# levje/TrackToLearn

Measured on AMD Instinct MI355X. Metric: streamline-steps/s at n_actor=262144, higher is better.
Workload: dtype f32

## Files before the change

tracktolearn_amd/csrc/ttl_hip.hip:

```cpp
#include <hip/hip_runtime.h>

#include <algorithm>
#include <atomic>
#include <chrono>
#include <cmath>
#include <cstdarg>
#include <cstdio>
#include <cstdlib>
#include <cstring>
#include <new>
#include <type_traits>

#include "ttl_hip.h"

#include "ttl_internal.h"

#include <map>
#include <mutex>

namespace {
thread_local char g_err[512] = "";
}

int ttl_detail_fail(int code, const char *fmt, ...) {
// ... 1117 lines not shown
    const size_t nb = (n + BLOCK - 1) / BLOCK + 1;
    size_t end = 0;
    const auto rows = [&](auto *&region, size_t count, size_t per_row, size_t align = 256) {
        region = base ? reinterpret_cast<std::remove_reference_t<decltype(region)>>(
                            static_cast<char *>(base) + end) : nullptr;
        end += align_up(count * per_row, align);
    };
    rows(P.stop, n, 1);
    rows(P.rank, n, sizeof(int));
    rows(P.surv_pos, n, sizeof(int));
    rows(P.row_dest, n, sizeof(int));
    rows(P.block_counts, nb, sizeof(int));
    rows(P.proc_rank, n, sizeof(int));
    rows(P.proc_counts, nb, sizeof(int));
    rows(e.proc[0], n, sizeof(int));
    rows(e.proc[1], n, sizeof(int));
    rows(P.head, n, 4 * sizeof(float));
    rows(P.slot_head, n, 4 * sizeof(float));
    rows(P.last2, n, 8 * sizeof(float));
    rows(P.pos_dest, n, 2 * sizeof(int));
    rows(P.stop_list, n, 2 * sizeof(int));
    rows(P.slot_dest, n, sizeof(int));
    rows(P.counts, 64, sizeof(int));
    const size_t order_bytes = ttl_detail_order_workspace_bytes(n);
    static_assert(sizeof(ActRecord) <= 256 && alignof(ActRecord) <= 8, "see above");
    e.order_ws_bytes = order_bytes - 256;
    rows(e.order_ws, order_bytes, 1, 1);
    e.act_rec = e.order_ws ? reinterpret_cast<ActRecord *>(e.order_ws + e.order_ws_bytes) : nullptr;
    rows(e.ord_rec, n, sizeof(int2));
    rows(e.ord_count[0], 1, ttl_detail_order_instep_count_bytes());
    rows(e.ord_count[1], 1, ttl_detail_order_instep_count_bytes());
    return end;
}

static int knob(const char *name, int unset) {
    const char *v = getenv(name);
    return v ? atoi(v) : unset;
}
static void ttl_env_read_knobs(ttl_env &e) {
    EnvParams &P = e.P;
    const int rider_kinds[4] = {0, 3, 1, 2};
    e.proc_min_rows = knob("TTL_ORDER_MIN_ROWS", 8192);
    e.instep = std::max(knob("TTL_ORDER_INSTEP", 2), 0);
    e.instep_after = knob("TTL_ORDER_INSTEP_AFTER", 0) != 0;
    e.tail_riders = rider_kinds[knob("TTL_TAIL_RIDERS", 1) & 3];
    e.state_kernel = knob("TTL_STATE_KERNEL", 4);
    P.slot_rec = e.state_kernel != 2;
    P.xcd_remap = knob("TTL_XCD_REMAP", 1);
    P.xcd_rot = knob("TTL_XCD_ROTATE", 0) & 7;
    P.store_flavour = knob("TTL_STORE_FLAVOUR", 0);
    e.fuse_small = knob("TTL_FUSE_SMALL", 1);
    P.fuse_max_rows = std::clamp(knob("TTL_FUSE_MAX_ROWS", 64 * BLOCK), BLOCK, TTL_FUSE_MAX_BLOCKS * BLOCK);
    P.persist_rows = knob("TTL_GATHER_PERSIST_ROWS", 0);
    e.tail_fused = knob("TTL_TAIL_FUSED", 1);
    e.tail_fused_max = std::min(knob("TTL_TAIL_FUSED_MAX_ROWS", 262144), TTL_TAIL_MAX_BLOCKS * BLOCK);
    e.local_sort = knob("TTL_LOCAL_SORT", 1);
    e.poll_counts = knob("TTL_POLL_COUNTS", 1);
}

static int64_t state_width(const ttl_env_desc &d) { return 7LL * d.n_coef + 3LL * d.n_dirs; }

static int *idx_of(const ttl_env *env, int ahead = 0) {
    return (env->cur ^ ahead) ? env->d.idx_b : env->d.idx_a;
}

static void order_holds(ttl_env *env, int n) { env->use_proc = 1, env->n_slots = n; }
static void order_dropped(ttl_env *env) { env->use_proc = 0; }
static void order_rearmed(ttl_env *env, bool installed, int n) {
    env->proc_cur = env->ord_parity = 0;
    installed ? order_holds(env, n) : order_dropped(env);
}
static void order_compacted(ttl_env *env) { env->n_slots = -1; }
static void order_rebuilt(ttl_env *env) { env->ord_parity ^= 1, env->n_slots = -1; }
static void order_swapped(ttl_env *env) { env->proc_cur ^= env->use_proc ? 1 : 0; }
static int order_len(const ttl_env *env, int rows) { return env->n_slots < 0 ? rows : env->n_slots; }

extern "C" {

const char *ttl_last_error(void) { return g_err; }
uint32_t ttl_abi_version(void) { return TTL_ABI_VERSION; }
size_t ttl_env_desc_size(void) { return sizeof(ttl_env_desc); }

size_t ttl_env_workspace_bytes(int32_t n_max) {
    ttl_env sized;
    return n_max < 0 ? 0 : ttl_env_carve(sized, (size_t)n_max, nullptr);
}

int64_t ttl_sh_volume_records(const int32_t *dim, int32_t layout) {
    if (!dim || dim[0] < 1 || dim[1] < 1 || dim[2] < 1) return 0;
    if (layout == TTL_SH_BRICK4)
        return (int64_t)((dim[0] + 3) / 4) * ((dim[1] + 3) / 4) * ((dim[2] + 3) / 4) * 64;
    return (int64_t)dim[0] * dim[1] * dim[2];
}

struct VmmBlock {
    hipMemGenericAllocationHandle_t handle;
    size_t size;
};
static std::mutex g_vmm_mutex;
static std::map<void *, VmmBlock> g_vmm_blocks;

static hipError_t vmm_alloc(int device, size_t bytes, void **out) {
    hipMemAllocationProp prop{};
    prop.type = hipMemAllocationTypePinned;
    prop.location.type = hipMemLocationTypeDevice;
    prop.location.id = device;
// ... 991 lines not shown
```

tracktolearn_amd/csrc/ttl_internal.h:

```cpp
#ifndef TTL_INTERNAL_H
#define TTL_INTERNAL_H
#include <hip/hip_runtime.h>

#include <cstdint>

#include "ttl_hip.h"

int ttl_detail_fail(int code, const char *fmt, ...) __attribute__((format(printf, 2, 3)));
#define fail ttl_detail_fail

#define HIP_TRY(expr)                                                        \
    do {                                                                     \
        hipError_t e_ = (expr);                                              \
        if (e_ != hipSuccess)                                                \
            return fail(TTL_ERR_HIP, "%s: %s", #expr, hipGetErrorString(e_)); \
    } while (0)

constexpr int TTL_BLOCK = 256;

struct EnvParams {
    int mode;
    int sh_dim[3];
    int n_coef;
    int coef_pitch;
    const float *sh;
    float sh_shift;
    int sh_brick;
    unsigned sh_sx, sh_sy;
    int mask_dim[3];
    const double *mask_coef;
    const uint8_t *mask_cls;
    double mask_thr;
    int peaks_dim[3];
    const float *peaks;
    int compute_reward;
    float align_w;
    int n_dirs;
    int max_nb_steps;
    double step64;
    float step32;
    float radius;
    int curv_enabled;
    float curv_dot_max;
    float *hist;
    int *flags;
    int *lengths;
    uint8_t *dones;
    uint8_t *stop;
    float *head;
    int *pos_dest;
    float *last2;
    int *rank;
    int *surv_pos;
    int *row_dest;
    int *stop_list;
    int *block_counts;
    int *proc_rank;
    int *proc_counts;
    float *slot_head;
    int *slot_dest;
    int slot_rec;
    int store_flavour;
    int xcd_remap;
    int xcd_rot;
    int *counts;
    int fuse_max_rows;
    int persist_rows;
};

constexpr int TTL_FUSE_MAX_BLOCKS = 256;

constexpr int TTL_FR_LIVE = 8;
constexpr int TTL_FR_SNAP = 16;
constexpr int TTL_FR_NOISE = 32;

__device__ __forceinline__ void philox4x32_10(uint32_t &c0, uint32_t &c1, uint32_t &c2,
                                              uint32_t &c3, uint32_t k0, uint32_t k1) {
#pragma unroll
    for (int r = 0; r < 10; ++r) {
        const uint32_t hi0 = __umulhi(0xD2511F53u, c0), lo0 = 0xD2511F53u * c0;
        const uint32_t hi1 = __umulhi(0xCD9E8D57u, c2), lo1 = 0xCD9E8D57u * c2;
        c0 = hi1 ^ c1 ^ k0;
        c1 = lo1;
        c2 = hi0 ^ c3 ^ k1;
        c3 = lo0;
        k0 += 0x9E3779B9u;
        k1 += 0xBB67AE85u;
    }
}

struct FreerunView {
    const int *live, *idx_a, *idx_b;
    int cap;
};
void ttl_detail_freerun_view(const ttl_env *env, FreerunView *out);

__device__ __forceinline__ unsigned vox_x(const EnvParams &P, int x) {
    return P.sh_brick ? (unsigned)(x >> 2) * P.sh_sx + (unsigned)(x & 3) * 16u
                      : (unsigned)x * P.sh_sx;
}
__device__ __forceinline__ unsigned vox_y(const EnvParams &P, int y) {
    return P.sh_brick ? (unsigned)(y >> 2) * P.sh_sy + (unsigned)(y & 3) * 4u
                      : (unsigned)y * P.sh_sy;
}
__device__ __forceinline__ unsigned vox_z(const EnvParams &P, int z) {
    return P.sh_brick ? (unsigned)(z >> 2) * 64u + (unsigned)(z & 3) : (unsigned)z;
}

__device__ __forceinline__ int step_row_dest(int order, int row, bool stop, int pos, int total) {
    int dest = row;
    if (order == TTL_ORDER_PARTITION) dest = stop ? total + (row - pos) : pos;
    return dest;
}

__device__ __forceinline__ int step_map_row(const EnvParams &P, int row, int g, bool stop,
                                            int pos, int total, int order, int n_pts,
                                            int *idx_next) {
    const int dest = step_row_dest(order, row, stop, pos, total);
    if (!stop) idx_next[pos] = g;
    if (stop && order == TTL_ORDER_PARTITION) P.lengths[g] = n_pts;
// ... 519 lines not shown
```

tracktolearn_amd/csrc/ttl_state.hip:

```cpp
#include <type_traits>

#include "ttl_internal.h"


namespace {
constexpr int BLOCK = TTL_BLOCK;

template <int LPS>
struct LaneGroups {
    static constexpr int PER_WAVE = 64 / LPS;
    static constexpr int PER_BLOCK = (BLOCK / 64) * PER_WAVE;
    static dim3 grid(int n_rows) { return dim3((n_rows + PER_BLOCK - 1) / PER_BLOCK); }

    int grp, sub;
    __device__ LaneGroups() {
        const int lane = threadIdx.x & 63;
        grp = lane / LPS;
        sub = lane - grp * LPS;
    }
    __device__ bool idle() const { return grp >= PER_WAVE; }
    __device__ int slot(int blk) const {
        return blk * PER_BLOCK + (threadIdx.x >> 6) * PER_WAVE + grp;
    }
};

__device__ __forceinline__ const float *history_of(const EnvParams &P, int g) {
    return P.hist + (size_t)g * (size_t)(P.max_nb_steps + 1) * 3;
}

struct seg3 {
    float x, y, z;
};
__device__ __forceinline__ seg3 dir_segment(const float *__restrict__ h, int n_seg, int j) {
    seg3 v{0.0f, 0.0f, 0.0f};
    if (j < n_seg) {
        const float *a = h + (n_seg - 1 - j) * 3;
        const float ax = a[0], ay = a[1], az = a[2];
        const float bx = a[3], by = a[4], bz = a[5];
        v = seg3{bx - ax, by - ay, bz - az};
    }
    return v;
}
__device__ __forceinline__ void put_segment(float *__restrict__ od, int j, seg3 v) {
    od[3 * j + 0] = v.x;
    od[3 * j + 1] = v.y;
    od[3 * j + 2] = v.z;
}

template <int LPS>
__global__ __launch_bounds__(BLOCK) void k_state(
    EnvParams P, const int *__restrict__ idx, const int *__restrict__ row_dest,
    const int *__restrict__ proc, int n_rows, int L, float *__restrict__ out,
    long long pitch) {
#pragma clang fp contract(fast)
    const LaneGroups<LPS> lanes;
    const int slot = lanes.slot(blockIdx.x), sub = lanes.sub;
    if (lanes.idle() || slot >= n_rows) return;
    const int row = proc ? proc[slot] : slot;
    if (row < 0) return;
    const int g = idx ? idx[row] : row;
    const int r = row_dest ? row_dest[row] : row;
    const float *h = history_of(P, g);
    const float px = h[(L - 1) * 3 + 0];
    const float py = h[(L - 1) * 3 + 1];
    const float pz = h[(L - 1) * 3 + 2];
    float *orow = out + (size_t)r * (size_t)pitch;
    const int C = P.n_coef;
    const int C4 = P.coef_pitch >> 2;
    const int X = P.sh_dim[0], Y = P.sh_dim[1], Z = P.sh_dim[2];
    const float4 *vol = reinterpret_cast<const float4 *>(P.sh);

    for (int c4 = sub; c4 < C4; c4 += LPS) {
#pragma unroll
        for (int k = 0; k < 7; ++k) {
            const float ox = (k == 1) ? P.radius : (k == 4) ? -P.radius : 0.0f;
            const float oy = (k == 2) ? P.radius : (k == 5) ? -P.radius : 0.0f;
// ... 36 lines not shown
    a.comp = a.comp + v3.comp * w3;                                          \
    a.comp = a.comp + v4.comp * w4;                                          \
    a.comp = a.comp + v5.comp * w5;                                          \
    a.comp = a.comp + v6.comp * w6;                                          \
    a.comp = a.comp + v7.comp * w7;
            TTL_ACC(x) TTL_ACC(y) TTL_ACC(z) TTL_ACC(w)
#undef TTL_ACC
            const int c = c4 * 4;
            float *o = orow + k * C + c;
            if (c + 0 < C) o[0] = a.x;
            if (c + 1 < C) o[1] = a.y;
            if (c + 2 < C) o[2] = a.z;
            if (c + 3 < C) o[3] = a.w;
        }
    }
    float *od = orow + 7 * C;
    const int n_seg = L - 1;
    for (int j = sub; j < P.n_dirs; j += LPS) put_segment(od, j, dir_segment(h, n_seg, j));
}

struct f4 {
    float x, y, z, w;
};
__device__ __forceinline__ f4 ld4(const char *base, unsigned byte_off) {
    const float4 v = *reinterpret_cast<const float4 *>(base + byte_off);
    return f4{v.x, v.y, v.z, v.w};
}
__device__ __forceinline__ f4 scale4(f4 a, float w) {
    return f4{a.x * w, a.y * w, a.z * w, a.w * w};
}
__device__ __forceinline__ f4 fma4(f4 a, float w, f4 c) {
    return f4{__builtin_fmaf(a.x, w, c.x), __builtin_fmaf(a.y, w, c.y),
              __builtin_fmaf(a.z, w, c.z), __builtin_fmaf(a.w, w, c.w)};
}
__device__ __forceinline__ f4 sel4(bool c, f4 a, f4 b) {
    return f4{c ? a.x : b.x, c ? a.y : b.y, c ? a.z : b.z, c ? a.w : b.w};
}
template <bool OUTER>
__device__ __forceinline__ f4 blend(f4 v00, f4 v01, f4 v10, f4 v11, float a0, float a1,
                                    float b0, float b1) {
    f4 r = OUTER ? fma4(v00, a0 * b0, scale4(v01, a0 * b1))
                 : fma4(v01, a0 * b1, scale4(v00, a0 * b0));
    r = fma4(v10, a1 * b0, r);
    return fma4(v11, a1 * b1, r);
}
template <bool MINUS>
__device__ __forceinline__ f4 lerp(f4 lo, f4 hi, float d) {
    return MINUS ? fma4(hi, d, scale4(lo, 1.0f - d)) : fma4(lo, 1.0f - d, scale4(hi, d));
}
struct AxisPoints {
    f4 centre, plus, minus;
};
__device__ __forceinline__ AxisPoints stencil_axis(
    const char *vol, const f4 (&lo)[4], const f4 (&hi)[4], const unsigned (&q)[4], unsigned below,
    unsigned above, float a0, float a1, float b0, float b1, bool dn, bool up, float d,
    float d_plus, float d_minus) {
    const f4 zero{0.f, 0.f, 0.f, 0.f};
    f4 s0 = zero, s3 = zero;
    if (dn)
        s0 = blend<true>(ld4(vol, below + q[0]), ld4(vol, below + q[1]), ld4(vol, below + q[2]),
                         ld4(vol, below + q[3]), a0, a1, b0, b1);
    if (up)
        s3 = blend<true>(ld4(vol, above + q[0]), ld4(vol, above + q[1]), ld4(vol, above + q[2]),
                         ld4(vol, above + q[3]), a0, a1, b0, b1);
    const f4 s1 = blend<false>(lo[0], lo[1], lo[2], lo[3], a0, a1, b0, b1);
    const f4 s2 = blend<false>(hi[0], hi[1], hi[2], hi[3], a0, a1, b0, b1);
    return AxisPoints{lerp<false>(s1, s2, d),
                      lerp<false>(sel4(up, s2, s1), sel4(up, s3, s2), d_plus),
                      lerp<true>(sel4(dn, s0, s1), sel4(dn, s1, s2), d_minus)};
}
__device__ __forceinline__ int clipi(int v, int n) { return min(max(v, 0), n - 1); }
typedef float v4f __attribute__((ext_vector_type(4)));
typedef v4f v4f_dword_aligned __attribute__((aligned(4)));
__device__ __forceinline__ float from_prev_lane(float v) {
    return __int_as_float(
        __builtin_amdgcn_update_dpp(0, __float_as_int(v), 0x111, 0xf, 0xf, false));
}
__device__ __forceinline__ void store16(float *o, v4f v, int flavour) {
    if (flavour == 0) {
        *reinterpret_cast<v4f_dword_aligned *>(o) = v;
    } else if (flavour == 1) {
        asm volatile("global_store_dwordx4 %0, %1, off sc1" : : "v"(o), "v"(v) : "memory");
    } else if (flavour == 2) {
        asm volatile("global_store_dwordx4 %0, %1, off nt" : : "v"(o), "v"(v) : "memory");
    } else {
        asm volatile("global_store_dwordx4 %0, %1, off sc0 sc1" : : "v"(o), "v"(v) : "memory");
    }
}

template <bool MERGE_TAIL>
__device__ __forceinline__ void put4(int flavour, float *o, f4 a, int c, int C) {
    if (MERGE_TAIL && (flavour & 8)) {
        const int rem = C & 3;
        const bool last = c + 3 >= C;
        v4f v{a.x, a.y, a.z, a.w};
        int back = 0;
        if (rem == 1) {
            const float py = from_prev_lane(a.y), pz = from_prev_lane(a.z), pw = from_prev_lane(a.w);
            if (last) v = v4f{py, pz, pw, a.x};
            back = last ? 3 : 0;
        } else if (rem == 2) {
            const float pz = from_prev_lane(a.z), pw = from_prev_lane(a.w);
            if (last) v = v4f{pz, pw, a.x, a.y};
            back = last ? 2 : 0;
        } else if (rem == 3) {
            const float pw = from_prev_lane(a.w);
            if (last) v = v4f{pw, a.x, a.y, a.z};
            back = last ? 1 : 0;
        }
        store16(o - back, v, flavour & 7);
        return;
    }
    if (MERGE_TAIL) {
        const f4 p{from_prev_lane(a.x), from_prev_lane(a.y), from_prev_lane(a.z),
                   from_prev_lane(a.w)};
        const int back = (c + 3 < C) ? 0 : 4 - (C - c);
        v4f v{a.x, a.y, a.z, a.w};
        if (back == 1) v = v4f{p.w, a.x, a.y, a.z};
        if (back == 2) v = v4f{p.z, p.w, a.x, a.y};
        if (back == 3) v = v4f{p.y, p.z, p.w, a.x};
        store16(o - back, v, flavour);
        return;
    }
    if (c + 3 < C) {
        store16(o, v4f{a.x, a.y, a.z, a.w}, flavour);
    } else {
        if (c + 0 < C) o[0] = a.x;
        if (c + 1 < C) o[1] = a.y;
        if (c + 2 < C) o[2] = a.z;
    }
}

template <int LPS, bool LOOP, bool MERGE_TAIL>
__device__ __forceinline__ void state_row_dd(const EnvParams &P, float px, float py,
                                             float pz, const float *__restrict__ h, int L,
                                             int sub, float *__restrict__ orow) {
    const seg3 first_dir = sub < P.n_dirs ? dir_segment(h, L - 1, sub) : seg3{0.0f, 0.0f, 0.0f};
    const int C = P.n_coef;
    const int C4 = P.coef_pitch >> 2;
    const int X = P.sh_dim[0], Y = P.sh_dim[1], Z = P.sh_dim[2];
    const char *vol = reinterpret_cast<const char *>(P.sh);
    const float rad = P.radius;

    float cxp = px + rad, cxm = px + (-rad);
    float cyp = py + rad, cym = py + (-rad);
    float czp = pz + rad, czm = pz + (-rad);
    if (P.sh_shift != 0.0f) {
        px += P.sh_shift; py += P.sh_shift; pz += P.sh_shift;
        cxp += P.sh_shift; cxm += P.sh_shift;
        cyp += P.sh_shift; cym += P.sh_shift;
        czp += P.sh_shift; czm += P.sh_shift;
    }
    const float fx = floorf(px), fy = floorf(py), fz = floorf(pz);
    const float dx = px - fx, dy = py - fy, dz = pz - fz;
    const float ex = 1.0f - dx, ey = 1.0f - dy, ez = 1.0f - dz;
    const float fxp = floorf(cxp), fxm = floorf(cxm);
    const float fyp = floorf(cyp), fym = floorf(cym);
    const float fzp = floorf(czp), fzm = floorf(czm);
    const float dxp = cxp - fxp, dxm = cxm - fxm;
    const float dyp = cyp - fyp, dym = cym - fym;
    const float dzp = czp - fzp, dzm = czm - fzm;
    const bool xup = fxp > fx, xdn = fxm < fx;
    const bool yup = fyp > fy, ydn = fym < fy;
    const bool zup = fzp > fz, zdn = fzm < fz;
    const int ix = (int)fminf(fmaxf(fx, -4.0f), (float)X + 4.0f);
    const int iy = (int)fminf(fmaxf(fy, -4.0f), (float)Y + 4.0f);
    const int iz = (int)fminf(fmaxf(fz, -4.0f), (float)Z + 4.0f);
    const unsigned rec = (unsigned)C4 * 16u;
    const unsigned x0 = vox_x(P, clipi(ix - 1, X)) * rec, x1 = vox_x(P, clipi(ix, X)) * rec,
                   x2 = vox_x(P, clipi(ix + 1, X)) * rec, x3 = vox_x(P, clipi(ix + 2, X)) * rec;
    const unsigned y0 = vox_y(P, clipi(iy - 1, Y)) * rec, y1 = vox_y(P, clipi(iy, Y)) * rec,
                   y2 = vox_y(P, clipi(iy + 1, Y)) * rec, y3 = vox_y(P, clipi(iy + 2, Y)) * rec;
    const unsigned z0 = vox_z(P, clipi(iz - 1, Z)) * rec, z1 = vox_z(P, clipi(iz, Z)) * rec,
                   z2 = vox_z(P, clipi(iz + 1, Z)) * rec, z3 = vox_z(P, clipi(iz + 2, Z)) * rec;
    for (int c4 = sub; c4 < C4; c4 += LPS) {
        const unsigned cb = (unsigned)c4 * 16u;
        const int c = c4 * 4;
        const unsigned qx[4] = {y1 + z1 + cb, y1 + z2 + cb, y2 + z1 + cb, y2 + z2 + cb};
        const unsigned qy[4] = {x1 + z1 + cb, x1 + z2 + cb, x2 + z1 + cb, x2 + z2 + cb};
        const unsigned qz[4] = {x1 + y1 + cb, x1 + y2 + cb, x2 + y1 + cb, x2 + y2 + cb};
        const f4 v000 = ld4(vol, x1 + qx[0]), v001 = ld4(vol, x1 + qx[1]);
        const f4 v010 = ld4(vol, x1 + qx[2]), v011 = ld4(vol, x1 + qx[3]);
        const f4 v100 = ld4(vol, x2 + qx[0]), v101 = ld4(vol, x2 + qx[1]);
        const f4 v110 = ld4(vol, x2 + qx[2]), v111 = ld4(vol, x2 + qx[3]);
        const AxisPoints ax = stencil_axis(vol, {v000, v001, v010, v011}, {v100, v101, v110, v111},
                                           qx, x0, x3, ey, dy, ez, dz, xdn, xup, dx, dxp, dxm);
        put4<MERGE_TAIL>(P.store_flavour, orow + 0 * C + c, ax.centre, c, C);
        put4<MERGE_TAIL>(P.store_flavour, orow + 1 * C + c, ax.plus, c, C);
        put4<MERGE_TAIL>(P.store_flavour, orow + 4 * C + c, ax.minus, c, C);
        const AxisPoints ay = stencil_axis(vol, {v000, v001, v100, v101}, {v010, v011, v110, v111},
                                           qy, y0, y3, ex, dx, ez, dz, ydn, yup, dy, dyp, dym);
        put4<MERGE_TAIL>(P.store_flavour, orow + 2 * C + c, ay.plus, c, C);
        put4<MERGE_TAIL>(P.store_flavour, orow + 5 * C + c, ay.minus, c, C);
        const AxisPoints az = stencil_axis(vol, {v000, v010, v100, v110}, {v001, v011, v101, v111},
                                           qz, z0, z3, ex, dx, ey, dy, zdn, zup, dz, dzp, dzm);
        put4<MERGE_TAIL>(P.store_flavour, orow + 3 * C + c, az.plus, c, C);
        put4<MERGE_TAIL>(P.store_flavour, orow + 6 * C + c, az.minus, c, C);
        if (!LOOP) break;
    }
    float *od = orow + 7 * C;
    if (sub < P.n_dirs) put_segment(od, sub, first_dir);
    for (int j = sub + LPS; j < P.n_dirs; j += LPS)
        put_segment(od, j, dir_segment(h, L - 1, j));
}

__device__ __forceinline__ void tail_rider(const EnvParams &P, const TailRiders &R, int wg) {
    if (wg < R.n_scatter) {
        extern __shared__ unsigned s_rider[];
        order_scatter_block(s_rider, wg, R.n_scatter, R.rec, R.n_slots, R.count, R.count_other,
                            R.bins, R.order_out);
        return;
    }
    wg -= R.n_scatter;
    const int i = wg * BLOCK + threadIdx.x;
    if (wg >= R.n_row_blocks || i >= R.n_active) return;
    step_map_row(P, i, R.idx[i], P.stop[i] != 0, R.row_base[wg] + P.rank[i], P.counts[0],
                 R.order, R.n_pts, R.idx_next);
}

__device__ __forceinline__ int xcd_block(const EnvParams &P, int blk, int nwg) {
    const int q = nwg >> 3, rr = nwg & 7, xcd = blk & 7;
    if (P.xcd_rot == 0)
        return (xcd < rr ? xcd * (q + 1) : rr * (q + 1) + (xcd - rr) * q) + (blk >> 3);
    const int mine = (xcd + P.xcd_rot) & 7;
    int start = 0;
    for (int r = 0; r < mine; ++r) start += q + ((((r - P.xcd_rot) & 7) < rr) ? 1 : 0);
    return start + (blk >> 3);
}

struct SlotRow {
    int g, r;
    float px, py, pz;
    const float *h;
};
__device__ __forceinline__ bool resolve_slot(const EnvParams &P, const int *__restrict__ idx,
                                             const int *__restrict__ row_dest,
                                             const int *__restrict__ proc, int slot, int L,
                                             SlotRow &s) {
    if (proc && idx && P.slot_rec) {
        const float4 hp = *reinterpret_cast<const float4 *>(P.slot_head + 4 * (size_t)slot);
        s = SlotRow{__float_as_int(hp.w), P.slot_dest[slot], hp.x, hp.y, hp.z, nullptr};
        if (s.r < 0) return false;
        s.h = history_of(P, s.g);
        return true;
    }
    const int row = proc ? proc[slot] : slot;
    if (row < 0) return false;
    s.g = idx ? idx[row] : row;
    s.r = row_dest ? row_dest[row] : row;
    s.h = history_of(P, s.g);
    if (idx) {
        const float4 hp = *reinterpret_cast<const float4 *>(P.head + 4 * (size_t)row);
        s.px = hp.x;
        s.py = hp.y;
        s.pz = hp.z;
    } else {
        s.px = s.h[(L - 1) * 3 + 0];
        s.py = s.h[(L - 1) * 3 + 1];
        s.pz = s.h[(L - 1) * 3 + 2];
    }
    return true;
}

template <int LPS, int MINW, bool LOOP, bool MERGE_TAIL>
__global__ __launch_bounds__(BLOCK, MINW) void k_state_dd(
    EnvParams P, const int *__restrict__ idx, const int *__restrict__ row_dest,
    const int *__restrict__ proc, int n_rows, int L, float *__restrict__ out,
    long long pitch, int n_vblocks, TailRiders riders) {
    if ((int)blockIdx.x >= n_vblocks) {
        tail_rider(P, riders, (int)blockIdx.x - n_vblocks);
        return;
    }
    const LaneGroups<LPS> lanes;
    if (lanes.idle()) return;
    for (int vb = blockIdx.x; vb < n_vblocks; vb += gridDim.x) {
        const int slot = lanes.slot(proc && P.xcd_remap ? xcd_block(P, vb, n_vblocks) : vb);
        SlotRow s;
        if (slot >= n_rows || !resolve_slot(P, idx, row_dest, proc, slot, L, s)) continue;
        state_row_dd<LPS, LOOP, MERGE_TAIL>(P, s.px, s.py, s.pz, s.h, L, lanes.sub,
                                            out + (size_t)s.r * (size_t)pitch);
    }
}

template <int LPS, bool MERGE_TAIL, bool FR>
__device__ __forceinline__ void prefix_state_body(
    const EnvParams &P, const int *__restrict__ idx, int *__restrict__ idx_next, int n_active,
    int n_blocks, int order, int n_pts, float *__restrict__ out, long long pitch,
    int *__restrict__ host_word, int seq, int cur) {
    __shared__ int s_before[TTL_FUSE_MAX_BLOCKS + 1];
    const int lane = threadIdx.x & 63;
    if (threadIdx.x < 64) {
        int c[4];
#pragma unroll
        for (int k = 0; k < 4; ++k)
            c[k] = 4 * lane + k < n_blocks ? P.block_counts[4 * lane + k] : 0;
        const int local = (c[0] + c[1]) + (c[2] + c[3]);
        int v = local;
#pragma unroll
        for (int off = 1; off < 64; off <<= 1) {
            const int t = __shfl_up(v, off);
            if (lane >= off) v += t;
        }
        int run = v - local;
#pragma unroll
        for (int k = 0; k < 4; ++k) {
            s_before[4 * lane + k] = run;
            run += c[k];
        }
        if (lane == 63) s_before[TTL_FUSE_MAX_BLOCKS] = v;
    }
    __syncthreads();
    const int total = s_before[TTL_FUSE_MAX_BLOCKS];
    if (blockIdx.x == 0 && threadIdx.x == 0) {
        if (FR) {
            int *live = P.counts + TTL_FR_LIVE;
            live[0] = total;
            live[1] = n_active > 0 ? n_pts : n_pts - 1;
            live[2] = n_active > 0 ? cur ^ 1 : cur;
            live[3] = seq;
        }
        step_publish_counts(P, total, n_active, host_word, seq);
    }
    const LaneGroups<LPS> lanes;
    const int row = lanes.slot(blockIdx.x), sub = lanes.sub;
    if (lanes.idle() || row >= n_active) return;
    const float4 hp = *reinterpret_cast<const float4 *>(P.head + 4 * (size_t)row);
    const int g = __float_as_int(hp.w);
    const bool stop = P.stop[row] != 0;
    const int pos = s_before[row >> 8] + P.rank[row];
    const int dest = step_row_dest(order, row, stop, pos, total);
    if (sub == 0) step_map_row(P, row, g, stop, pos, total, order, n_pts, idx_next);
    state_row_dd<LPS, false, MERGE_TAIL>(P, hp.x, hp.y, hp.z, history_of(P, g), n_pts, sub,
                                         out + (size_t)dest * (size_t)pitch);
}

template <int LPS, bool MERGE_TAIL>
__global__ __launch_bounds__(BLOCK, 4) void k_prefix_state(
    EnvParams P, const int *__restrict__ idx, int *__restrict__ idx_next, int n_active,
    int n_blocks, int order, int n_pts, float *__restrict__ out, long long pitch,
    int *__restrict__ host_word, int seq) {
    prefix_state_body<LPS, MERGE_TAIL, false>(P, idx, idx_next, n_active, n_blocks, order,
                                              n_pts, out, pitch, host_word, seq, 0);
}

template <int LPS, bool MERGE_TAIL>
__global__ __launch_bounds__(BLOCK, 4) void k_prefix_state_fr(
    EnvParams P, int *__restrict__ idx_a, int *__restrict__ idx_b, int n_blocks,
    float *__restrict__ out, long long pitch, int *__restrict__ host_word) {
    const int *snap = P.counts + TTL_FR_SNAP;
    const int n_active = snap[0], L = snap[1], cur = snap[2], seq = snap[3] + 1;
    if (snap[4]) {
        if (blockIdx.x == 0 && threadIdx.x == 0) {
            P.counts[TTL_FR_LIVE + 3] = seq;
            if (host_word)
                __hip_atomic_store(host_word + 2, seq, __ATOMIC_RELEASE, __HIP_MEMORY_SCOPE_SYSTEM);
        }
        return;
    }
    prefix_state_body<LPS, MERGE_TAIL, true>(P, cur ? idx_b : idx_a, cur ? idx_a : idx_b,
                                             n_active, n_blocks, TTL_ORDER_PARTITION, L + 1,
                                             out, pitch, host_word, seq, cur);
}

template <int MAX_LPS, class F>
void for_lanes_per_streamline(const EnvParams &P, F &&f) {
    const int C4 = P.coef_pitch >> 2;
    const bool tail_straddles = C4 == 9 && (P.n_coef & 3);
    if (C4 <= 4) f(std::integral_constant<int, 4>{});
    else if (C4 <= 8) f(std::integral_constant<int, 8>{});
    else if (C4 <= 12 && !tail_straddles) f(std::integral_constant<int, 12>{});
    else if (MAX_LPS == 16 || C4 <= 16) f(std::integral_constant<int, 16>{});
    else f(std::integral_constant<int, MAX_LPS>{});
}

bool dedupe_applies(const EnvParams &P) {
    const size_t vol_bytes = ttl_detail_sh_records(P) * P.coef_pitch * sizeof(float);
    return P.radius > 0.0f && P.radius < 1.0f && vol_bytes < (1ull << 32);
}

}

bool ttl_detail_can_fuse_tail(const EnvParams &P, int n_active) {
    const int C4 = P.coef_pitch >> 2;
    return n_active <= P.fuse_max_rows && dedupe_applies(P) && C4 <= 16 && P.n_coef >= 4;
}

int ttl_detail_launch_fused_tail(const EnvParams &P, const int *idx, int *idx_next,
                                 int n_active, int order, int n_pts, float *out,
                                 int64_t pitch, int *host_word, int seq, hipStream_t s) {
    const int n_blocks = (n_active + BLOCK - 1) / BLOCK;
    for_lanes_per_streamline<16>(P, [&](auto lps) {
        constexpr int LPS = decltype(lps)::value;
        hipLaunchKernelGGL((k_prefix_state<LPS, true>), LaneGroups<LPS>::grid(n_active), dim3(BLOCK), 0,
                           s, P, idx, idx_next, n_active, n_blocks, order, n_pts, out,
                           (long long)pitch, host_word, seq);
    });
    HIP_TRY(hipGetLastError());
    return TTL_OK;
}

int ttl_detail_launch_fused_tail_fr(const EnvParams &P, int *idx_a, int *idx_b, int n_cap,
                                    float *out, int64_t pitch, int *host_word,
                                    hipStream_t s) {
    const int n_blocks = (n_cap + BLOCK - 1) / BLOCK;
    for_lanes_per_streamline<16>(P, [&](auto lps) {
        constexpr int LPS = decltype(lps)::value;
        hipLaunchKernelGGL((k_prefix_state_fr<LPS, true>), LaneGroups<LPS>::grid(n_cap), dim3(BLOCK), 0,
                           s, P, idx_a, idx_b, n_blocks, out, (long long)pitch, host_word);
    });
    HIP_TRY(hipGetLastError());
    return TTL_OK;
}

bool ttl_detail_state_dedupes(const EnvParams &P, int state_kernel) {
    return state_kernel != 0 && dedupe_applies(P);
}

int ttl_detail_launch_state(const EnvParams &P, int state_kernel, const int *idx,
                            const int *row_dest, const int *proc, int n_rows, int L,
                            float *out, int64_t pitch, hipStream_t s,
                            const TailRiders *riders) {
    const bool dedupe = ttl_detail_state_dedupes(P, state_kernel);
    const TailRiders R = riders ? *riders : TailRiders{};
    const int n_riders = R.n_scatter + R.n_row_blocks;
    const size_t lds = R.n_scatter ? ttl_detail_order_scatter_lds(R.bins) : 0;
    if (n_riders && (!dedupe || P.persist_rows > 0 || lds > TTL_RIDER_MAX_LDS))
        return fail(TTL_ERR_INVALID, "state gather: this launch cannot carry riders");
    for_lanes_per_streamline<32>(P, [&](auto lps) {
        constexpr int LPS = decltype(lps)::value;
        const int n_vb = (int)LaneGroups<LPS>::grid(n_rows).x;
        const int resident = 1024;
        const bool persist = dedupe && n_rows <= P.persist_rows && n_vb > resident;
        const dim3 grid(persist ? resident : n_vb + n_riders);
        if (!dedupe)
            hipLaunchKernelGGL((k_state<LPS>), grid, dim3(BLOCK), 0, s, P, idx, row_dest, proc,
                               n_rows, L, out, (long long)pitch);
        else if constexpr (LPS < 32) {
            if (P.n_coef >= 4 && state_kernel != 3)
                hipLaunchKernelGGL((k_state_dd<LPS, 4, false, true>), grid, dim3(BLOCK), lds, s, P,
                                   idx, row_dest, proc, n_rows, L, out, (long long)pitch, n_vb, R);
            else
                hipLaunchKernelGGL((k_state_dd<LPS, 4, false, false>), grid, dim3(BLOCK), lds, s, P,
                                   idx, row_dest, proc, n_rows, L, out, (long long)pitch, n_vb, R);
        } else {
            hipLaunchKernelGGL((k_state_dd<LPS, 2, true, false>), grid, dim3(BLOCK), lds, s, P, idx,
                               row_dest, proc, n_rows, L, out, (long long)pitch, n_vb, R);
        }
    });
    HIP_TRY(hipGetLastError());
    return TTL_OK;
}
```

Baseline: 909.5 million.

## Restage state gather row to cut register pressure and pin waves per SIMD

Measured after the change: 912.5 million (median of 4 runs). About the same (+0.3%).

```diff
diff --git a/profiles/state_occupancy_resources.py b/profiles/state_occupancy_resources.py
--- /dev/null
+++ b/profiles/state_occupancy_resources.py
@@ -0,0 +1,124 @@
+#!/usr/bin/env python
+import argparse
+import importlib.util
+import os
+import re
+import subprocess
+import sys
+import tempfile
+
+ROOT = os.path.dirname(os.path.dirname(os.path.abspath(__file__)))
+TABLE = os.path.join(ROOT, 'profiles', 'state_occupancy_resource_usage.md')
+UNIT = 'tracktolearn_amd/csrc/ttl_state.hip'
+COLUMNS = ('SGPRs', 'SGPRs spilled', 'VGPRs', 'VGPRs spilled', 'scratch B/lane',
+           'waves/SIMD', 'LDS B/block')
+_REMARK = {'TotalSGPRs': 'SGPRs', 'SGPRs Spill': 'SGPRs spilled', 'VGPRs': 'VGPRs',
+           'VGPRs Spill': 'VGPRs spilled', 'ScratchSize': 'scratch B/lane',
+           'Occupancy': 'waves/SIMD', 'LDS Size': 'LDS B/block'}
+
+
+def _build_module():
+    spec = importlib.util.spec_from_file_location(
+        'ttl_csrc_build', os.path.join(ROOT, 'tracktolearn_amd', 'csrc', 'build.py'))
+    mod = importlib.util.module_from_spec(spec)
+    spec.loader.exec_module(mod)
+    return mod
+
+
+def kernel_name(mangled):
+    m = re.match(r'_ZN12_GLOBAL__N_1(\d+)', mangled)
+    if not m:
+        return mangled
+    start = m.end()
+    name = mangled[start:start + int(m.group(1))]
+    rest = mangled[start + int(m.group(1)):]
+    args = []
+    if rest.startswith('I'):
+        for kind, value in re.findall(r'L([ib])(n?\d+)E', rest[1:rest.index('EE') + 1]):
+            args.append(('false', 'true')[int(value)] if kind == 'b' else value.replace('n', '-'))
+    return f'{name}<{", ".join(args)}>' if args else name
+
+
+def report(tree=ROOT):
+    build = _build_module()
+    flags = [f for f in build.FLAGS if f not in ('-shared', '-fPIC')]
+    with tempfile.TemporaryDirectory() as tmp:
+        cmd = [build.find_hipcc()] + flags + [
+            '-Rpass-analysis=kernel-resource-usage', '--cuda-device-only',
+            '-I', os.path.join(tree, 'include'), '-I', os.path.join(tree, 'tracktolearn_amd', 'csrc'),
+            '-c', os.path.join(tree, UNIT), '-o', os.path.join(tmp, 'ttl_state.o')]
+        err = subprocess.run(cmd, check=True, stderr=subprocess.PIPE, text=True).stderr
+    kernels, cur = {}, None
+    for line in err.splitlines():
+        m = re.search(r'remark: +(.*?)(?: \[-Rpass-analysis=kernel-resource-usage\])?$', line)
+        if not m:
+            continue
+        text = m.group(1)
+        m = re.match(r'Function Name: (\S+)', text)
+        if m:
+            cur = kernels.setdefault(kernel_name(m.group(1)), {})
+            continue
+        m = re.match(r'([A-Za-z ]+?)(?: \[[^\]]*\])?: (\d+)$', text)
+        if m and cur is not None and m.group(1) in _REMARK:
+            cur[_REMARK[m.group(1)]] = int(m.group(2))
+    return kernels
+
+
+def table(kernels):
+    lines = ['| kernel | ' + ' | '.join(COLUMNS) + ' |', '|---' * (len(COLUMNS) + 1) + '|']
+    for name, row in kernels.items():
+        lines.append(f'| `{name}` | ' + ' | '.join(str(row[c]) for c in COLUMNS) + ' |')
+    return '\n'.join(lines)
+
+
+def read_table(heading, path=TABLE):
+    kernels, inside = {}, False
+    with open(path) as f:
+        for line in f:
+            if line.startswith('## '):
+                inside = line[3:].strip() == heading
+            m = re.match(r'\| `([^`]+)` \|(.*)\|\s*$', line)
+            if inside and m:
+                kernels[m.group(1)] = dict(zip(COLUMNS, (int(v) for v in m.group(2).split('|'))))
+    return kernels
+
+
+def parent_tree(rev, tmp):
+    for path in ('include', 'tracktolearn_amd/csrc'):
+        tar = subprocess.run(['git', '-C', ROOT, 'archive', rev, path], check=True,
+                             stdout=subprocess.PIPE).stdout
+        subprocess.run(['tar', '-x', '-C', tmp], input=tar, check=True)
+    return tmp
+
+
+HEADER = '''# State gather: registers, scratch and waves per SIMD (DESIGN 3.1, 4.1)
+
+The compiler's report (`-Rpass-analysis=kernel-resource-usage`) of every kernel of
+`tracktolearn_amd/csrc/ttl_state.hip`, compiled alone and device side only with the flags of
+`tracktolearn_amd/csrc/build.py`; written by `profiles/state_occupancy_resources.py`, runs without
+a GPU.  "Parent" is the commit before the row of `state_row_dd` was restated in four stages (the
+centre cell reduced to its six blended slices at once, then one axis at a time with its own
+geometry); "This tree" is the source next to this file.  The second template argument of
+`k_state_dd` is the waves per SIMD the instantiation is held to (`amdgpu_waves_per_eu`, both
+bounds; `TTL_GATHER_WAVES` picks 4, 5 or 6 for the one-column gather): where the body needs fewer
+registers than that bound allows, the kernel descriptor is padded to it, so "waves/SIMD" is what
+the hardware will keep resident.  `tests/test_state_kernel_resources.py` holds this tree to the
+table below: no instantiation may gain scratch, and the 5-wave gather has none.
+'''
+
+
+def main():
+    ap = argparse.ArgumentParser(description=__doc__.split('\n')[0])
+    ap.add_argument('--parent', default='HEAD~1', help='revision of the parent tree')
+    args = ap.parse_args()
+    with tempfile.TemporaryDirectory() as tmp:
+        parent = report(parent_tree(args.parent, tmp))
+    rev = subprocess.run(['git', '-C', ROOT, 'rev-parse', '--short', args.parent], check=True,
+                         stdout=subprocess.PIPE, text=True).stdout.strip()
+    with open(TABLE, 'w') as f:
+        f.write(f'{HEADER}\n## Parent\n\n(`{rev}`)\n\n{table(parent)}\n\n## This tree\n\n{table(report())}\n')
+    print(TABLE)
+
+
+if __name__ == '__main__':
+    sys.exit(main())
diff --git a/tracktolearn_amd/csrc/ttl_hip.hip b/tracktolearn_amd/csrc/ttl_hip.hip
--- a/tracktolearn_amd/csrc/ttl_hip.hip
+++ b/tracktolearn_amd/csrc/ttl_hip.hip
@@ -1193,6 +1193,7 @@
     e.fuse_small = knob("TTL_FUSE_SMALL", 1);
     P.fuse_max_rows = std::clamp(knob("TTL_FUSE_MAX_ROWS", 64 * BLOCK), BLOCK, TTL_FUSE_MAX_BLOCKS * BLOCK);
     P.persist_rows = knob("TTL_GATHER_PERSIST_ROWS", 0);
+    P.gather_waves = std::clamp(knob("TTL_GATHER_WAVES", 4), 4, 6);
     e.tail_fused = knob("TTL_TAIL_FUSED", 1);
     e.tail_fused_max = std::min(knob("TTL_TAIL_FUSED_MAX_ROWS", 262144), TTL_TAIL_MAX_BLOCKS * BLOCK);
     e.local_sort = knob("TTL_LOCAL_SORT", 1);
diff --git a/tracktolearn_amd/csrc/ttl_internal.h b/tracktolearn_amd/csrc/ttl_internal.h
--- a/tracktolearn_amd/csrc/ttl_internal.h
+++ b/tracktolearn_amd/csrc/ttl_internal.h
@@ -66,6 +66,7 @@
     int *counts;
     int fuse_max_rows;
     int persist_rows;
+    int gather_waves;
 };
 
 constexpr int TTL_FUSE_MAX_BLOCKS = 256;
diff --git a/tracktolearn_amd/csrc/ttl_state.hip b/tracktolearn_amd/csrc/ttl_state.hip
--- a/tracktolearn_amd/csrc/ttl_state.hip
+++ b/tracktolearn_amd/csrc/ttl_state.hip
@@ -12,16 +12,15 @@
     static constexpr int PER_BLOCK = (BLOCK / 64) * PER_WAVE;
     static dim3 grid(int n_rows) { return dim3((n_rows + PER_BLOCK - 1) / PER_BLOCK); }
 
-    int grp, sub;
-    __device__ LaneGroups() {
-        const int lane = threadIdx.x & 63;
+    int wave, grp, sub;
+    __device__ explicit LaneGroups(int tid = threadIdx.x) {
+        const int lane = tid & 63;
+        wave = tid >> 6;
         grp = lane / LPS;
         sub = lane - grp * LPS;
     }
     __device__ bool idle() const { return grp >= PER_WAVE; }
-    __device__ int slot(int blk) const {
-        return blk * PER_BLOCK + (threadIdx.x >> 6) * PER_WAVE + grp;
-    }
+    __device__ int slot(int blk) const { return blk * PER_BLOCK + wave * PER_WAVE + grp; }
 };
 
 __device__ __forceinline__ const float *history_of(const EnvParams &P, int g) {
@@ -164,9 +163,9 @@
     f4 centre, plus, minus;
 };
 __device__ __forceinline__ AxisPoints stencil_axis(
-    const char *vol, const f4 (&lo)[4], const f4 (&hi)[4], const unsigned (&q)[4], unsigned below,
-    unsigned above, float a0, float a1, float b0, float b1, bool dn, bool up, float d,
-    float d_plus, float d_minus) {
+    const char *vol, f4 s1, f4 s2, const unsigned (&q)[4], unsigned below, unsigned above,
+    float a0, float a1, float b0, float b1, bool dn, bool up, float d, float d_plus,
+    float d_minus) {
     const f4 zero{0.f, 0.f, 0.f, 0.f};
     f4 s0 = zero, s3 = zero;
     if (dn)
@@ -175,8 +174,6 @@
     if (up)
         s3 = blend<true>(ld4(vol, above + q[0]), ld4(vol, above + q[1]), ld4(vol, above + q[2]),
                          ld4(vol, above + q[3]), a0, a1, b0, b1);
-    const f4 s1 = blend<false>(lo[0], lo[1], lo[2], lo[3], a0, a1, b0, b1);
-    const f4 s2 = blend<false>(hi[0], hi[1], hi[2], hi[3], a0, a1, b0, b1);
     return AxisPoints{lerp<false>(s1, s2, d),
                       lerp<false>(sel4(up, s2, s1), sel4(up, s3, s2), d_plus),
                       lerp<true>(sel4(dn, s0, s1), sel4(dn, s1, s2), d_minus)};
@@ -243,77 +240,131 @@
     }
 }
 
+struct AxisGeom {
+    unsigned o[4];
+    float d, e, d_plus, d_minus;
+    bool up, dn;
+};
+template <int AXIS>
+__device__ __forceinline__ unsigned vox_axis(const EnvParams &P, int v) {
+    const bool brick = P.sh_brick != 0;
+    const unsigned stride = AXIS == 0 ? P.sh_sx : AXIS == 1 ? P.sh_sy : brick ? 64u : 1u;
+    const unsigned within = (unsigned)(v & 3) * (AXIS == 0 ? 16u : AXIS == 1 ? 4u : 1u);
+    return (unsigned)(brick ? v >> 2 : v) * stride + (brick ? within : 0u);
+}
+template <int AXIS, bool OUTER>
+__device__ __forceinline__ AxisGeom axis_geom(const EnvParams &P, float p, unsigned rec) {
+    const int n = P.sh_dim[AXIS];
+    float cp = p + P.radius, cm = p + (-P.radius);
+    if (P.sh_shift != 0.0f) {
+        p += P.sh_shift;
+        cp += P.sh_shift;
+        cm += P.sh_shift;
+    }
+    const float f = floorf(p);
+    AxisGeom g;
+    g.d = p - f;
+    g.e = 1.0f - g.d;
+    const int i = (int)fminf(fmaxf(f, -4.0f), 1.0e9f);
+    g.o[1] = vox_axis<AXIS>(P, clipi(i, n)) * rec;
+    g.o[2] = vox_axis<AXIS>(P, clipi(i + 1, n)) * rec;
+    if (OUTER) {
+        const float fp = floorf(cp), fm = floorf(cm);
+        g.d_plus = cp - fp;
+        g.d_minus = cm - fm;
+        g.up = fp > f;
+        g.dn = fm < f;
+        g.o[0] = vox_axis<AXIS>(P, clipi(i - 1, n)) * rec;
+        g.o[3] = vox_axis<AXIS>(P, clipi(i + 2, n)) * rec;
+    }
+    return g;
+}
+__device__ __forceinline__ void rederive_from(float &x, float &y, float &z) {
+    asm("" : "+v"(x), "+v"(y), "+v"(z));
+}
+__device__ __forceinline__ void settle(f4 &a) {
+    asm volatile("" : "+v"(a.x), "+v"(a.y), "+v"(a.z), "+v"(a.w));
+}
+
 template <int LPS, bool LOOP, bool MERGE_TAIL>
 __device__ __forceinline__ void state_row_dd(const EnvParams &P, float px, float py,
-                                             float pz, const float *__restrict__ h, int L,
-                                             int sub, float *__restrict__ orow) {
-    const seg3 first_dir = sub < P.n_dirs ? dir_segment(h, L - 1, sub) : seg3{0.0f, 0.0f, 0.0f};
+                                             float pz, int g, int L, int sub,
+                                             float *__restrict__ orow) {
     const int C = P.n_coef;
     const int C4 = P.coef_pitch >> 2;
-    const int X = P.sh_dim[0], Y = P.sh_dim[1], Z = P.sh_dim[2];
+    const seg3 first_dir = sub < C4 && sub < P.n_dirs ? dir_segment(history_of(P, g), L - 1, sub)
+                                                      : seg3{0.0f, 0.0f, 0.0f};
     const char *vol = reinterpret_cast<const char *>(P.sh);
-    const float rad = P.radius;
-
-    float cxp = px + rad, cxm = px + (-rad);
-    float cyp = py + rad, cym = py + (-rad);
-    float czp = pz + rad, czm = pz + (-rad);
-    if (P.sh_shift != 0.0f) {
-        px += P.sh_shift; py += P.sh_shift; pz += P.sh_shift;
-        cxp += P.sh_shift; cxm += P.sh_shift;
-        cyp += P.sh_shift; cym += P.sh_shift;
-        czp += P.sh_shift; czm += P.sh_shift;
-    }
-    const float fx = floorf(px), fy = floorf(py), fz = floorf(pz);
-    const float dx = px - fx, dy = py - fy, dz = pz - fz;
-    const float ex = 1.0f - dx, ey = 1.0f - dy, ez = 1.0f - dz;
-    const float fxp = floorf(cxp), fxm = floorf(cxm);
-    const float fyp = floorf(cyp), fym = floorf(cym);
-    const float fzp = floorf(czp), fzm = floorf(czm);
-    const float dxp = cxp - fxp, dxm = cxm - fxm;
-    const float dyp = cyp - fyp, dym = cym - fym;
-    const float dzp = czp - fzp, dzm = czm - fzm;
-    const bool xup = fxp > fx, xdn = fxm < fx;
-    const bool yup = fyp > fy, ydn = fym < fy;
-    const bool zup = fzp > fz, zdn = fzm < fz;
-    const int ix = (int)fminf(fmaxf(fx, -4.0f), (float)X + 4.0f);
-    const int iy = (int)fminf(fmaxf(fy, -4.0f), (float)Y + 4.0f);
-    const int iz = (int)fminf(fmaxf(fz, -4.0f), (float)Z + 4.0f);
     const unsigned rec = (unsigned)C4 * 16u;
-    const unsigned x0 = vox_x(P, clipi(ix - 1, X)) * rec, x1 = vox_x(P, clipi(ix, X)) * rec,
-                   x2 = vox_x(P, clipi(ix + 1, X)) * rec, x3 = vox_x(P, clipi(ix + 2, X)) * rec;
-    const unsigned y0 = vox_y(P, clipi(iy - 1, Y)) * rec, y1 = vox_y(P, clipi(iy, Y)) * rec,
-                   y2 = vox_y(P, clipi(iy + 1, Y)) * rec, y3 = vox_y(P, clipi(iy + 2, Y)) * rec;
-    const unsigned z0 = vox_z(P, clipi(iz - 1, Z)) * rec, z1 = vox_z(P, clipi(iz, Z)) * rec,
-                   z2 = vox_z(P, clipi(iz + 1, Z)) * rec, z3 = vox_z(P, clipi(iz + 2, Z)) * rec;
     for (int c4 = sub; c4 < C4; c4 += LPS) {
         const unsigned cb = (unsigned)c4 * 16u;
         const int c = c4 * 4;
-        const unsigned qx[4] = {y1 + z1 + cb, y1 + z2 + cb, y2 + z1 + cb, y2 + z2 + cb};
-        const unsigned qy[4] = {x1 + z1 + cb, x1 + z2 + cb, x2 + z1 + cb, x2 + z2 + cb};
-        const unsigned qz[4] = {x1 + y1 + cb, x1 + y2 + cb, x2 + y1 + cb, x2 + y2 + cb};
-        const f4 v000 = ld4(vol, x1 + qx[0]), v001 = ld4(vol, x1 + qx[1]);
-        const f4 v010 = ld4(vol, x1 + qx[2]), v011 = ld4(vol, x1 + qx[3]);
-        const f4 v100 = ld4(vol, x2 + qx[0]), v101 = ld4(vol, x2 + qx[1]);
-        const f4 v110 = ld4(vol, x2 + qx[2]), v111 = ld4(vol, x2 + qx[3]);
-        const AxisPoints ax = stencil_axis(vol, {v000, v001, v010, v011}, {v100, v101, v110, v111},
-                                           qx, x0, x3, ey, dy, ez, dz, xdn, xup, dx, dxp, dxm);
-        put4<MERGE_TAIL>(P.store_flavour, orow + 0 * C + c, ax.centre, c, C);
-        put4<MERGE_TAIL>(P.store_flavour, orow + 1 * C + c, ax.plus, c, C);
-        put4<MERGE_TAIL>(P.store_flavour, orow + 4 * C + c, ax.minus, c, C);
-        const AxisPoints ay = stencil_axis(vol, {v000, v001, v100, v101}, {v010, v011, v110, v111},
-                                           qy, y0, y3, ex, dx, ez, dz, ydn, yup, dy, dyp, dym);
-        put4<MERGE_TAIL>(P.store_flavour, orow + 2 * C + c, ay.plus, c, C);
-        put4<MERGE_TAIL>(P.store_flavour, orow + 5 * C + c, ay.minus, c, C);
-        const AxisPoints az = stencil_axis(vol, {v000, v010, v100, v110}, {v001, v011, v101, v111},
-                                           qz, z0, z3, ex, dx, ey, dy, zdn, zup, dz, dzp, dzm);
-        put4<MERGE_TAIL>(P.store_flavour, orow + 3 * C + c, az.plus, c, C);
-        put4<MERGE_TAIL>(P.store_flavour, orow + 6 * C + c, az.minus, c, C);
+        f4 sx1, sx2, sy1, sy2, sz1, sz2;
+        {
+            const AxisGeom gx = axis_geom<0, false>(P, px, rec);
+            const AxisGeom gy = axis_geom<1, false>(P, py, rec);
+            const AxisGeom gz = axis_geom<2, false>(P, pz, rec);
+            const unsigned q[4] = {gy.o[1] + gz.o[1] + cb, gy.o[1] + gz.o[2] + cb,
+                                   gy.o[2] + gz.o[1] + cb, gy.o[2] + gz.o[2] + cb};
+            const f4 v000 = ld4(vol, gx.o[1] + q[0]), v001 = ld4(vol, gx.o[1] + q[1]);
+            const f4 v010 = ld4(vol, gx.o[1] + q[2]), v011 = ld4(vol, gx.o[1] + q[3]);
+            const f4 v100 = ld4(vol, gx.o[2] + q[0]), v101 = ld4(vol, gx.o[2] + q[1]);
+            const f4 v110 = ld4(vol, gx.o[2] + q[2]), v111 = ld4(vol, gx.o[2] + q[3]);
+            sx1 = blend<false>(v000, v001, v010, v011, gy.e, gy.d, gz.e, gz.d);
+            sx2 = blend<false>(v100, v101, v110, v111, gy.e, gy.d, gz.e, gz.d);
+            sy1 = blend<false>(v000, v001, v100, v101, gx.e, gx.d, gz.e, gz.d);
+            sy2 = blend<false>(v010, v011, v110, v111, gx.e, gx.d, gz.e, gz.d);
+            sz1 = blend<false>(v000, v010, v100, v110, gx.e, gx.d, gy.e, gy.d);
+            sz2 = blend<false>(v001, v011, v101, v111, gx.e, gx.d, gy.e, gy.d);
+            settle(sx1), settle(sx2), settle(sy1), settle(sy2), settle(sz1), settle(sz2);
+        }
+        if (c4 == sub && sub < P.n_dirs) put_segment(orow + 7 * C, sub, first_dir);
+        {
+            rederive_from(px, py, pz);
+            const AxisGeom gx = axis_geom<0, true>(P, px, rec);
+            const AxisGeom gy = axis_geom<1, false>(P, py, rec);
+            const AxisGeom gz = axis_geom<2, false>(P, pz, rec);
+            const unsigned q[4] = {gy.o[1] + gz.o[1] + cb, gy.o[1] + gz.o[2] + cb,
+                                   gy.o[2] + gz.o[1] + cb, gy.o[2] + gz.o[2] + cb};
+            const AxisPoints a = stencil_axis(vol, sx1, sx2, q, gx.o[0], gx.o[3], gy.e, gy.d, gz.e,
+                                              gz.d, gx.dn, gx.up, gx.d, gx.d_plus, gx.d_minus);
+            put4<MERGE_TAIL>(P.store_flavour, orow + (unsigned)(0 * C + c), a.centre, c, C);
+            put4<MERGE_TAIL>(P.store_flavour, orow + (unsigned)(1 * C + c), a.plus, c, C);
+            put4<MERGE_TAIL>(P.store_flavour, orow + (unsigned)(4 * C + c), a.minus, c, C);
+        }
+        {
+            rederive_from(px, py, pz);
+            const AxisGeom gx = axis_geom<0, false>(P, px, rec);
+            const AxisGeom gy = axis_geom<1, true>(P, py, rec);
+            const AxisGeom gz = axis_geom<2, false>(P, pz, rec);
+            const unsigned q[4] = {gx.o[1] + gz.o[1] + cb, gx.o[1] + gz.o[2] + cb,
+                                   gx.o[2] + gz.o[1] + cb, gx.o[2] + gz.o[2] + cb};
+            const AxisPoints a = stencil_axis(vol, sy1, sy2, q, gy.o[0], gy.o[3], gx.e, gx.d, gz.e,
+                                              gz.d, gy.dn, gy.up, gy.d, gy.d_plus, gy.d_minus);
+            put4<MERGE_TAIL>(P.store_flavour, orow + (unsigned)(2 * C + c), a.plus, c, C);
+            put4<MERGE_TAIL>(P.store_flavour, orow + (unsigned)(5 * C + c), a.minus, c, C);
+        }
+        {
+            rederive_from(px, py, pz);
+            const AxisGeom gx = axis_geom<0, false>(P, px, rec);
+            const AxisGeom gy = axis_geom<1, false>(P, py, rec);
+            const AxisGeom gz = axis_geom<2, true>(P, pz, rec);
+            const unsigned q[4] = {gx.o[1] + gy.o[1] + cb, gx.o[1] + gy.o[2] + cb,
+                                   gx.o[2] + gy.o[1] + cb, gx.o[2] + gy.o[2] + cb};
+            const AxisPoints a = stencil_axis(vol, sz1, sz2, q, gz.o[0], gz.o[3], gx.e, gx.d, gy.e,
+                                              gy.d, gz.dn, gz.up, gz.d, gz.d_plus, gz.d_minus);
+            put4<MERGE_TAIL>(P.store_flavour, orow + (unsigned)(3 * C + c), a.plus, c, C);
+            put4<MERGE_TAIL>(P.store_flavour, orow + (unsigned)(6 * C + c), a.minus, c, C);
+        }
         if (!LOOP) break;
     }
-    float *od = orow + 7 * C;
-    if (sub < P.n_dirs) put_segment(od, sub, first_dir);
-    for (int j = sub + LPS; j < P.n_dirs; j += LPS)
-        put_segment(od, j, dir_segment(h, L - 1, j));
+    const int j0 = sub < C4 ? sub + LPS : sub;
+    if (j0 < P.n_dirs) {
+        asm("" : "+v"(g));
+        const float *h = history_of(P, g);
+        float *od = orow + 7 * C;
+        for (int j = j0; j < P.n_dirs; j += LPS) put_segment(od, j, dir_segment(h, L - 1, j));
+    }
 }
 
 __device__ __forceinline__ void tail_rider(const EnvParams &P, const TailRiders &R, int wg) {
@@ -343,7 +394,6 @@
 struct SlotRow {
     int g, r;
     float px, py, pz;
-    const float *h;
 };
 __device__ __forceinline__ bool resolve_slot(const EnvParams &P, const int *__restrict__ idx,
                                              const int *__restrict__ row_dest,
@@ -351,31 +401,29 @@
                                              SlotRow &s) {
     if (proc && idx && P.slot_rec) {
         const float4 hp = *reinterpret_cast<const float4 *>(P.slot_head + 4 * (size_t)slot);
-        s = SlotRow{__float_as_int(hp.w), P.slot_dest[slot], hp.x, hp.y, hp.z, nullptr};
-        if (s.r < 0) return false;
-        s.h = history_of(P, s.g);
-        return true;
+        s = SlotRow{__float_as_int(hp.w), P.slot_dest[slot], hp.x, hp.y, hp.z};
+        return s.r >= 0;
     }
     const int row = proc ? proc[slot] : slot;
     if (row < 0) return false;
     s.g = idx ? idx[row] : row;
     s.r = row_dest ? row_dest[row] : row;
-    s.h = history_of(P, s.g);
     if (idx) {
         const float4 hp = *reinterpret_cast<const float4 *>(P.head + 4 * (size_t)row);
         s.px = hp.x;
         s.py = hp.y;
         s.pz = hp.z;
     } else {
-        s.px = s.h[(L - 1) * 3 + 0];
-        s.py = s.h[(L - 1) * 3 + 1];
-        s.pz = s.h[(L - 1) * 3 + 2];
+        const float *h = history_of(P, s.g);
+        s.px = h[(L - 1) * 3 + 0];
+        s.py = h[(L - 1) * 3 + 1];
+        s.pz = h[(L - 1) * 3 + 2];
     }
     return true;
 }
 
-template <int LPS, int MINW, bool LOOP, bool MERGE_TAIL>
-__global__ __launch_bounds__(BLOCK, MINW) void k_state_dd(
+template <int LPS, int WAVES, bool LOOP, bool MERGE_TAIL>
+__global__ __launch_bounds__(BLOCK) __attribute__((amdgpu_waves_per_eu(WAVES, WAVES))) void k_state_dd(
     EnvParams P, const int *__restrict__ idx, const int *__restrict__ row_dest,
     const int *__restrict__ proc, int n_rows, int L, float *__restrict__ out,
     long long pitch, int n_vblocks, TailRiders riders) {
@@ -383,13 +431,15 @@
         tail_rider(P, riders, (int)blockIdx.x - n_vblocks);
         return;
     }
-    const LaneGroups<LPS> lanes;
-    if (lanes.idle()) return;
+    if (LaneGroups<LPS>().idle()) return;
     for (int vb = blockIdx.x; vb < n_vblocks; vb += gridDim.x) {
+        int tid = threadIdx.x;
+        asm("" : "+v"(tid));
+        const LaneGroups<LPS> lanes(tid);
         const int slot = lanes.slot(proc && P.xcd_remap ? xcd_block(P, vb, n_vblocks) : vb);
         SlotRow s;
         if (slot >= n_rows || !resolve_slot(P, idx, row_dest, proc, slot, L, s)) continue;
-        state_row_dd<LPS, LOOP, MERGE_TAIL>(P, s.px, s.py, s.pz, s.h, L, lanes.sub,
+        state_row_dd<LPS, LOOP, MERGE_TAIL>(P, s.px, s.py, s.pz, s.g, L, lanes.sub,
                                             out + (size_t)s.r * (size_t)pitch);
     }
 }
@@ -442,7 +492,7 @@
     const int pos = s_before[row >> 8] + P.rank[row];
     const int dest = step_row_dest(order, row, stop, pos, total);
     if (sub == 0) step_map_row(P, row, g, stop, pos, total, order, n_pts, idx_next);
-    state_row_dd<LPS, false, MERGE_TAIL>(P, hp.x, hp.y, hp.z, history_of(P, g), n_pts, sub,
+    state_row_dd<LPS, false, MERGE_TAIL>(P, hp.x, hp.y, hp.z, g, n_pts, sub,
                                          out + (size_t)dest * (size_t)pitch);
 }
 
@@ -548,12 +598,21 @@
             hipLaunchKernelGGL((k_state<LPS>), grid, dim3(BLOCK), 0, s, P, idx, row_dest, proc,
                                n_rows, L, out, (long long)pitch);
         else if constexpr (LPS < 32) {
-            if (P.n_coef >= 4 && state_kernel != 3)
-                hipLaunchKernelGGL((k_state_dd<LPS, 4, false, true>), grid, dim3(BLOCK), lds, s, P,
-                                   idx, row_dest, proc, n_rows, L, out, (long long)pitch, n_vb, R);
-            else
-                hipLaunchKernelGGL((k_state_dd<LPS, 4, false, false>), grid, dim3(BLOCK), lds, s, P,
-                                   idx, row_dest, proc, n_rows, L, out, (long long)pitch, n_vb, R);
+            const bool merge = P.n_coef >= 4 && state_kernel != 3;
+            auto launch = [&](auto kernel) {
+                hipLaunchKernelGGL(kernel, grid, dim3(BLOCK), lds, s, P, idx, row_dest, proc, n_rows,
+                                   L, out, (long long)pitch, n_vb, R);
+            };
+            if (P.gather_waves == 6) {
+                if (merge) launch(k_state_dd<LPS, 6, false, true>);
+                else launch(k_state_dd<LPS, 6, false, false>);
+            } else if (P.gather_waves == 5) {
+                if (merge) launch(k_state_dd<LPS, 5, false, true>);
+                else launch(k_state_dd<LPS, 5, false, false>);
+            } else {
+                if (merge) launch(k_state_dd<LPS, 4, false, true>);
+                else launch(k_state_dd<LPS, 4, false, false>);
+            }
         } else {
             hipLaunchKernelGGL((k_state_dd<LPS, 2, true, false>), grid, dim3(BLOCK), lds, s, P, idx,
                                row_dest, proc, n_rows, L, out, (long long)pitch, n_vb, R);
```
